# sisl/NeRFSafetyValidation

Measured on AMD Instinct MI355X. Metric: rendered_samples_per_sec, higher is better.
Workload: dtype f16; 1 GPU; Stonehenge 800x800 synthetic, hashgrid L=16 F=2 T=2^19 + ffmlp(64,2)/(64,3), fp16, occupancy-grid ray marching (run_cuda eval path, BASELINE configs[1]); rays_per_frame=640000, bound=2, cascade=2, frames_in_flight=3, fused_reference_rounding=True, parallelism=single GPU, rccl_ranks=1

## Files before the change

nerfsafetyvalidation_amd/csrc/render_fused.hip:

```cpp
#include <hip/hip_fp16.h>
#include <math.h>
#include <string.h>

#include <atomic>
#include <mutex>

#include "ngp_common.hpp"

namespace ngp {

typedef _Float16 half8 __attribute__((ext_vector_type(8)));
typedef _Float16 half2v __attribute__((ext_vector_type(2)));
typedef _Float16 half4 __attribute__((ext_vector_type(4)));
typedef float f32x4 __attribute__((ext_vector_type(4)));

constexpr int kWaves = 8;
constexpr int kThreads = kWaves * 64;
constexpr int kWavesPerSimd = 4;
constexpr int kCh = 2;
constexpr int kSlots = 64 * kCh;
constexpr size_t kLinMaxBytes = 4u << 20;
constexpr size_t kCoarseMaxBytes = 8192;
constexpr int kLookahead = 4;
constexpr int kRing = 8;
// ... 2026 lines not shown
    Pcg32 rng;
    const uint32_t* coarse;
    uint32_t coarse_words;
    const uint32_t* bitfield_lin;
    uint32_t log_grid;
    uint32_t block_jump;
    uint32_t* sample_hash;
    unsigned long long* stamps;
    float2* march_samples;
    uint8_t* march_counts;
    uint32_t wave_slots;
    uint32_t n_rays;
    uint32_t pre_verdict;
    uint32_t wave_march_max;
    uint32_t cell_runs;
};

__host__ __device__ __forceinline__ uint32_t item_width(uint32_t n_alive, uint32_t wave_slots) {
    return n_alive >= 64u * wave_slots ? 64u : (n_alive >= 32u * wave_slots ? 32u : 16u);
}
__device__ __forceinline__ void truncate_launch(Ctl& c, const uint32_t* exhausted, uint32_t N) {
    if (!c.spec) return;
    const uint32_t q = c.spec, K = c.n_step / q;
    uint32_t alive = c.n_alive, ok = K;
    for (uint32_t j = 0; j < K; j++) {
        if (alive == 0) break;
        const uint32_t want_q = N / alive;
        if (j > 0 && (want_q < 1 ? 1u : (want_q > 8 ? 8u : want_q)) != q) { ok = j; break; }
        alive -= exhausted[j] < alive ? exhausted[j] : alive;
    }
// ... 13 lines not shown
    float t[kSlots], dt[kSlots], sig[kSlots];
    uint32_t rg[kSlots], b[kSlots];
    uint16_t list[kSlots];
    float od[64][6];
};

__device__ __forceinline__ void dump_row(const RenderArgs& ra, uint32_t entry, int32_t ray, uint32_t n_step, uint32_t k, float sg, float r,
                                         float g, float b) {
    if (ra.dump_rec) {
        ra.dump_rec[(size_t)ray * 8 + k] = make_float4(sg, r, g, b);
    } else {
        const size_t row = (size_t)entry * n_step + k;
        ra.last_sigmas[row] = sg;
        ra.last_rgbs[row * 3] = r; ra.last_rgbs[row * 3 + 1] = g; ra.last_rgbs[row * 3 + 2] = b;
    }
}

__device__ __forceinline__ void march_ahead_wave(const RenderArgs& ra, float bound, const Ctl& ctl, const uint32_t* coarse) {
    const uint32_t lane = threadIdx.x & 63u;
    const uint32_t entry = blockIdx.x * 4u + (threadIdx.x >> 6);
    if (entry >= ctl.n_alive) return;
    const uint32_t n_step = ctl.n_step, spec = ctl.spec;
    const int32_t ray = ra.alive_in[entry];
    Dda dda;
    dda.init(ra.rays_o + (size_t)ray * 3, ra.rays_d + (size_t)ray * 3, ra.bitfield, bound, 0.0f, ra.max_steps, ra.cascade, ra.grid_size);
    dda.init_lin(ra.bitfield_lin, ra.log_grid, ra.block_jump != 0);
    const float t_c = ra.rays_t[ray], far = ra.fars[ray];
    float t_march = t_c;
    if (ra.perturb) {
        Pcg32 rng = ra.rng;
// ... 162 lines not shown
    if (ctl.spec) {
        uint32_t* exhausted = reinterpret_cast<uint32_t*>(smem);
        if (threadIdx.x < kSpecK) {
            uint32_t d = 0;
            for (int sh = 0; sh < kDeathShards; sh++) d += ra.death_shards[(size_t)kDeathShards * kSpecK + sh * kSpecK + threadIdx.x];
            exhausted[threadIdx.x] = d;
        }
        __syncthreads();
        truncate_launch(ctl, exhausted, ra.n_rays);
        __syncthreads();
    }
    const uint32_t n_alive = ctl.n_alive, n_step = ctl.n_step;
    const uint32_t spec = ctl.spec;
    const uint32_t W = item_width(n_alive, ra.wave_slots);
    const uint32_t n_chunks = (n_alive + W - 1) / W;

    const size_t w_bytes = net_w_bytes_f16(na);
    _Float16* Wlds = reinterpret_cast<_Float16*>(smem);
    LevelTab* lt = reinterpret_cast<LevelTab*>(smem + w_bytes);
    WaveSlab* slabs = reinterpret_cast<WaveSlab*>(smem + w_bytes + sizeof(LevelTab));
    stage_block(na, lv, Wlds, lt, w_bytes);

    const uint32_t lane = threadIdx.x & 63, wid = threadIdx.x >> 6, c = lane & 15;
    WaveSlab& S = slabs[wid];
    unsigned long long ts0 = 0, ts1 = 0;
#define NGP_STAMP(idx)                                                                  \
    if (ra.stamps) {                                                                    \
        ts1 = __builtin_amdgcn_s_memtime();                                             \
        if (lane == 0) atomicAdd(ra.stamps + (idx), ts1 - ts0);                         \
        ts0 = ts1;                                                                      \
// ... 127 lines not shown
                }
                if (lane < 16 && valid) {
                    S.sig[slot] = na.density_scale * sg;
                    S.rg[slot] = (uint32_t)__builtin_bit_cast(uint16_t, (_Float16)r) | ((uint32_t)__builtin_bit_cast(uint16_t, (_Float16)g) << 16);
                    S.b[slot] = (uint32_t)__builtin_bit_cast(uint16_t, (_Float16)b);
                }
            }
            if (ra.stamps && lane == 0) {
                atomicAdd(ra.stamps + 8, sub_a); atomicAdd(ra.stamps + 9, sub_b); atomicAdd(ra.stamps + 10, sub_n); atomicAdd(ra.stamps + 11, sub_f);
            }
            NGP_STAMP(1)
            if (running) {
                uint32_t k = 0;
                for (; k < cnt; k++) {
                    const uint32_t slot = lane * kCh + k;
                    const float dt = S.dt[slot];
                    const float t_after = S.t[slot] + dt;
                    const float delta1 = t_after - last_t;
                    last_t = t_after;
                    const float sg = S.sig[slot];
                    const uint32_t rg = S.rg[slot];
                    const float sr = (float)__builtin_bit_cast(_Float16, (uint16_t)(rg & 0xffffu));
                    const float sgc = (float)__builtin_bit_cast(_Float16, (uint16_t)(rg >> 16));
                    const float sb = (float)__builtin_bit_cast(_Float16, (uint16_t)(S.b[slot] & 0xffffu));
                    const float alpha = 1.0f - expf(-sg * dt);
                    const float T = 1 - ws;
                    const float w = alpha * T;
                    ws += w;
                    t_c += delta1;
                    dep = fmaf(w, t_c, dep);
                    cr = fmaf(w, sr, cr); cg = fmaf(w, sgc, cg); cb = fmaf(w, sb, cb);
                    if (spec && (s0 + k + 1) % spec == 0) last_t = t_c;
                    if ((double)T < 1e-4) break;
                }
                steps_done += k;
                if (k < want) running = false;
            } else if (do_march && cnt) {
                last_t = S.t[lane * kCh + cnt - 1] + S.dt[lane * kCh + cnt - 1];
            }
            if (ra.last_sigmas && active && !spec) {
                for (uint32_t k = 0; k < want; k++) {
                    const uint32_t slot = lane * kCh + k;
                    if (k < cnt)
                        dump_row(ra, entry, ray, n_step, s0 + k, S.sig[slot], (float)__builtin_bit_cast(_Float16, (uint16_t)(S.rg[slot] & 0xffffu)),
                                 (float)__builtin_bit_cast(_Float16, (uint16_t)(S.rg[slot] >> 16)),
                                 (float)__builtin_bit_cast(_Float16, (uint16_t)(S.b[slot] & 0xffffu)));
                    else
                        dump_row(ra, entry, ray, n_step, s0 + k, ra.pad_sigma, ra.pad_r, ra.pad_g, ra.pad_b);
                }
            }
            NGP_STAMP(2)
            if (!ra.last_sigmas && !__any(running)) break;
        }

        const bool survive = active && running && steps_done == n_step;
        if (active) {
            if (survive) ra.rays_t[ray] = t_c;
            if (ra.sample_hash) {
                const uint32_t entered = (spec && !survive) ? (steps_done / spec + 1) * spec : n_step;
                const uint32_t n_hash = emitted < entered ? emitted : entered;
                uint32_t hsh = ra.sample_hash[ray];
                float lm = t_start, gtc = t_c0;
                for (uint32_t i = 0; i < n_hash; i++) {
                    const float2 v = marched[(size_t)i * 64];
                    const float ta = v.x + v.y, d1 = ta - lm;
                    lm = ta;
                    hsh = (hsh ^ __float_as_uint(v.y)) * 16777619u;
                    hsh = (hsh ^ __float_as_uint(d1)) * 16777619u;
                    gtc += d1;
                    if (spec && (i + 1) % spec == 0) lm = gtc;
                }
                ra.sample_hash[ray] = hsh;
            }
            ra.weights_sum[ray] = ws; ra.depth[ray] = dep;
            ra.image[(size_t)ray * 3] = cr; ra.image[(size_t)ray * 3 + 1] = cg; ra.image[(size_t)ray * 3 + 2] = cb;
        }
        const bool slow = ra.sort_slow && survive && slow_next;
        const unsigned long long ball_f = __ballot(survive && !slow), ball_s = __ballot(survive && slow);
        const unsigned long long lt_mask = (1ull << lane) - 1ull;
        if (survive && !slow) ra.staging[(size_t)first_entry + (uint32_t)__popcll(ball_f & lt_mask)] = ray;
        if (survive && slow) ra.staging[(size_t)first_entry + W - 1 - (uint32_t)__popcll(ball_s & lt_mask)] = ray;
        if (lane == 0) ra.chunk_count[chunk] = (uint32_t)__popcll(ball_f) | ((uint32_t)__popcll(ball_s) << 16);
        if (spec) {
            const uint32_t ds = ((blockIdx.x * kWaves + wid) % kDeathShards) * kSpecK;
            for (uint32_t m = 0; m < n_step / spec; m++) {
                const uint32_t cdead = (uint32_t)__popcll(__ballot(active && !survive && steps_done / spec == m));
                if (lane == 0 && cdead) atomicAdd(&ra.death_shards[ds + m], cdead);
            }
        }
        {
            const uint32_t entered = (spec && !survive) ? (steps_done / spec + 1) * spec : n_step;
            uint32_t rm = active ? (emitted < entered ? emitted : entered) : 0u;
#pragma unroll
            for (int off = 32; off > 0; off >>= 1) rm += __shfl_xor(rm, off, 64);
            wave_samples = rm;
        }
        wave_total += wave_samples;
        if (ra.dump_iter && active) ra.dump_iter[ray] = ctl.iters;
        if (ra.last_sigmas && !ra.dump_rec && !spec && chunk == n_chunks - 1) {
            for (uint32_t i = lane; i < 128; i += 64) {
                const size_t row = (size_t)n_alive * n_step + i;
                ra.last_sigmas[row] = ra.pad_sigma;
// ... 10 lines not shown
                                               uint32_t call_tag = 0) {
    if (!host_slot) return;
    if (n.done && fin) {
        const unsigned long long tag = (unsigned long long)(0x8000u | (call_tag & 0x7FFFu)) << 48;
        __hip_atomic_store(fin + 0, tag | (n.samples_marched & 0xFFFFFFFFFFFFull), __ATOMIC_RELAXED, __HIP_MEMORY_SCOPE_SYSTEM);
        __hip_atomic_store(fin + 1, tag | (n.samples_slots & 0xFFFFFFFFFFFFull), __ATOMIC_RELAXED, __HIP_MEMORY_SCOPE_SYSTEM);
        __hip_atomic_store(fin + 2, tag | ((unsigned long long)(n.iters & 0xFFFFFFu) << 24) | (n.rollbacks & 0xFFFFFFu), __ATOMIC_RELAXED,
                           __HIP_MEMORY_SCOPE_SYSTEM);
        __hip_atomic_store(fin + 3, tag | ((unsigned long long)n.last_n_alive << 8) | (n.last_n_step & 0xFFu), __ATOMIC_RELAXED,
                           __HIP_MEMORY_SCOPE_SYSTEM);
    }
    const unsigned long long w = ((unsigned long long)seq << 32) | ((unsigned long long)(n.done ? 1u : 0u) << 31) | (n.n_alive & 0x7FFFFFFFu);
    __hip_atomic_store(host_slot, w, __ATOMIC_RELAXED, __HIP_MEMORY_SCOPE_SYSTEM);
}

__global__ void __launch_bounds__(256) k_render_compact(const Ctl* __restrict__ cur, Ctl* __restrict__ nxt, const int32_t* __restrict__ staging,
                                                         const uint32_t* __restrict__ chunk_count, int32_t* __restrict__ alive_out, uint32_t N,
                                                         uint32_t max_steps, const unsigned long long* __restrict__ stat_shards,
                                                         QueueHeads* __restrict__ nxt_heads, unsigned long long* __restrict__ host_slot, uint32_t seq,
                                                         const uint32_t* __restrict__ death_shards, uint32_t spec_allowed, const int32_t* __restrict__ alive_in,
                                                         const float4* __restrict__ backup, float* __restrict__ rays_t, float* __restrict__ weights_sum,
                                                         float* __restrict__ depth, float* __restrict__ image, uint32_t* __restrict__ sample_hash,
                                                         unsigned long long* stat_shards_rw, uint32_t* __restrict__ death_next, uint32_t wave_slots,
                                                         uint32_t cap_mid_max, uint32_t cap_hi, unsigned long long* __restrict__ fin_host, uint32_t call_tag) {
    __shared__ uint32_t red[3][4];
    __shared__ uint32_t off_f[9], off_s[9];
    Ctl c = *cur;
    if (c.done) {
        if (blockIdx.x == 0 && threadIdx.x == 0) {
            *nxt = c;
            publish_status(host_slot, c, seq, fin_host, call_tag);
        }
        return;
    }
    const uint32_t W = item_width(c.n_alive, wave_slots);
    const uint32_t n_chunks = (c.n_alive + W - 1) / W;
    const uint32_t n_blocks = (n_chunks + 7) / 8;
    const uint32_t g = blockIdx.x;
    if (g >= n_blocks) return;
// ... 18 lines not shown
            const uint32_t q = c.spec, K = c.n_step / q;
            uint32_t alive = c.n_alive;
            keep = K;
            for (uint32_t j = 0; j < K; j++) {
                if (alive == 0) break;
                const uint32_t want_q = N / alive;
                if (j > 0 && (want_q < 1 ? 1u : (want_q > 8 ? 8u : want_q)) != q) { bad = 1; keep = j; break; }
                alive -= deaths[j];
                if ((spec_allowed & 2u) && alive == 0) { bad = 1; keep = j; break; }
            }
        }
        verdict_bad = bad;
        verdict_keep = keep;
    }
    __syncthreads();
    if (verdict_bad) {
        for (uint32_t e = first * W + threadIdx.x; e < (first + 8) * W && e < c.n_alive; e += 256) {
            const int32_t ray = alive_in[e];
            const float4 a = backup[(size_t)ray * 2], b = backup[(size_t)ray * 2 + 1];
            rays_t[ray] = a.x; weights_sum[ray] = a.y; depth[ray] = a.z;
            if (sample_hash) sample_hash[ray] = __float_as_uint(a.w);
            image[(size_t)ray * 3] = b.x; image[(size_t)ray * 3 + 1] = b.y; image[(size_t)ray * 3 + 2] = b.z;
            alive_out[e] = ray;
        }
        if (g == n_blocks - 1 && threadIdx.x == 0) {
            Ctl n = c;
            n.rollbacks = c.rollbacks + 1;
            if (verdict_keep >= 2 && !(spec_allowed & 4u)) {
                n.spec = c.spec;
                n.n_step = verdict_keep * c.spec;
                n.backoff = 0;
                for (uint32_t i = 0; i < kDeathWords; i++) death_next[i] = 0;
            } else {
                n.spec = 0;
                const uint32_t ns = c.n_alive ? N / c.n_alive : 8;
                n.n_step = ns < 1 ? 1 : (ns > 8 ? 8 : ns);
                n.backoff = 2;
            }
            for (int i = 0; i < kStatShards; i++) stat_shards_rw[i] = 0ull;
            *nxt = n;
            for (int i = 0; i < 8; i++) nxt_heads->head[i][0] = 0;
            publish_status(host_slot, n, seq, fin_host, call_tag);
        }
        return;
    }
    uint32_t pf = 0, ps = 0, tf = 0;
    for (uint32_t j = threadIdx.x; j < n_chunks; j += 256) {
        const uint32_t v = chunk_count[j];
        tf += v >> 16;
        if (j < first) { pf += v & 0xffffu; ps += v >> 16; }
    }
#pragma unroll
    for (int off = 32; off > 0; off >>= 1) {
        pf += __shfl_down(pf, off, 64);
// ... 14 lines not shown
    const uint32_t prefix_f = red[0][0] + red[0][1] + red[0][2] + red[0][3];
    const uint32_t prefix_s = red[1][0] + red[1][1] + red[1][2] + red[1][3];
    const uint32_t total_s = red[2][0] + red[2][1] + red[2][2] + red[2][3];
    const uint32_t lane = threadIdx.x & 63, w = threadIdx.x >> 6;
#pragma unroll
    for (uint32_t h = 0; h < 2; h++) {
        const uint32_t ci = w * 2 + h;
        const uint32_t nf = off_f[ci + 1] - off_f[ci], ns = off_s[ci + 1] - off_s[ci];
        if (lane < ns) alive_out[prefix_s + off_s[ci] + lane] = staging[(size_t)(first + ci) * W + W - 1 - lane];
        if (lane < nf) alive_out[total_s + prefix_f + off_f[ci] + lane] = staging[(size_t)(first + ci) * W + lane];
    }
    unsigned long long marched = threadIdx.x < (uint32_t)kStatShards ? stat_shards_rw[threadIdx.x] : 0ull;
#pragma unroll
    for (int off = 32; off > 0; off >>= 1) marched += __shfl_down(marched, off, 64);
    if (g == n_blocks - 1 && threadIdx.x == 0) {
        Ctl n = c;
        n.samples_marched = c.samples_marched + marched;
        for (int i = 0; i < kStatShards; i++) stat_shards_rw[i] = 0ull;
        n.n_alive = total_s + prefix_f + off_f[8];
        uint32_t recent = c.n_alive - n.n_alive;
        if (!c.spec) {
            n.last_n_alive = c.n_alive;
            n.last_n_step = c.n_step;
            n.iters = c.iters + 1;
            n.samples_slots = c.samples_slots + (unsigned long long)c.n_alive * c.n_step;
            n.step = c.step + c.n_step;
        } else {
            const uint32_t q = c.spec, K = c.n_step / q;
            uint32_t alive = c.n_alive, d_last = 0, d_prev = 0;
            unsigned long long slots = c.samples_slots;
            uint32_t it = 0;
            for (uint32_t j = 0; j < K; j++) {
                if (alive == 0) break;
                slots += (unsigned long long)alive * q;
                it++;
                n.last_n_alive = alive;
                n.last_n_step = q;
                alive -= deaths[j];
                d_prev = d_last;
                d_last = deaths[j];
            }
            recent = d_last > d_prev ? d_last : d_prev;
            n.iters = c.iters + it;
            n.samples_slots = slots;
            n.step = c.step + it * q;
        }
        uint32_t ns = n.n_alive ? N / n.n_alive : 8;
        n.n_step = ns < 1 ? 1 : (ns > 8 ? 8 : ns);
        n.done = (n.n_alive == 0 || n.step >= max_steps) ? 1 : 0;
        n.spec = 0;
        if (n.backoff) n.backoff--;
        else if (spec_allowed && !n.done && n.n_step <= kSpecMaxQ && (n.n_step == 8 || n.n_alive > N / (n.n_step + 1))) {
            const uint32_t q = n.n_step;
            const bool own_last = (spec_allowed & 2u) != 0;
            uint32_t room = (max_steps - n.step) / q;
            if (own_last && room) room--;
            const uint32_t headroom = n.n_alive - (q == 8 ? 0u : N / (q + 1)) - 1;
            uint32_t sq = 0;
            while ((unsigned long long)(sq + 1) * (sq + 1) <= recent) sq++;
            const unsigned long long rate = (unsigned long long)recent + 4ull * sq + 16ull;
            const uint32_t safety_x2 = (spec_allowed >> 8) ? (spec_allowed >> 8) : kSpecSafetyX2;
            uint32_t K = (uint32_t)((unsigned long long)headroom * 2u / (safety_x2 * rate));
            const uint32_t cap_mid = 8u * q < cap_mid_max ? 8u * q : cap_mid_max;
            const uint32_t cap_samples = q == 1 ? 8u : (q <= 4 ? cap_mid : cap_hi);
            const uint32_t capK = cap_samples / q < kSpecK ? cap_samples / q : kSpecK;
            K = (q == 8 && !own_last) ? capK : (K < capK ? K : capK);
            K = K < room ? K : room;
            if (K >= 2) { n.spec = q; n.n_step = K * q; }
        }
        if (n.spec)
            for (uint32_t i = 0; i < kDeathWords; i++) death_next[i] = 0;
        *nxt = n;
        for (int i = 0; i < 8; i++) nxt_heads->head[i][0] = 0;
        publish_status(host_slot, n, seq, fin_host, call_tag);
    }
}

__global__ void __launch_bounds__(256) k_render_init(uint32_t N, const float* __restrict__ nears, float* __restrict__ rays_t,
                                                      int32_t* __restrict__ alive, float* __restrict__ weights_sum, float* __restrict__ depth,
                                                      float* __restrict__ image, Ctl* __restrict__ ctl, uint32_t max_steps,
                                                      uint32_t* __restrict__ sample_hash, unsigned long long* __restrict__ stat_shards,
                                                      QueueHeads* __restrict__ heads, uint32_t* __restrict__ death_shards, uint32_t spec_allowed,
                                                      uint32_t tile_w) {
    const uint32_t n = blockIdx.x * 256 + threadIdx.x;
    if (n < (uint32_t)kStatShards) stat_shards[n] = 0ull;
    if (n < 2u * kDeathWords) death_shards[n] = 0;
    if (n < 16) heads[n >> 3].head[n & 7][0] = 0;
    if (n < N) {
        if (sample_hash) sample_hash[n] = 2166136261u;
        uint32_t first = n;
        if (tile_w) {
            const uint32_t t = n >> 4, in = n & 15u, per_row = tile_w >> 2;
            first = ((t / per_row) * 4u + (in >> 2)) * tile_w + (t % per_row) * 4u + (in & 3u);
        }
        alive[n] = (int32_t)first;
        rays_t[n] = nears[n];
        weights_sum[n] = 0; depth[n] = 0;
        image[(size_t)n * 3] = 0; image[(size_t)n * 3 + 1] = 0; image[(size_t)n * 3 + 2] = 0;
    }
    if (n == 0) {
// ... 81 lines not shown
}

using namespace ngp;

struct ngp_render_ctx {
    uint32_t max_rays = 0;
    uint32_t frame_width = 0;
    int32_t* alive[2] = {nullptr, nullptr};
    int32_t* staging = nullptr;
    uint32_t* chunk_count = nullptr;
    float* rays_t = nullptr;
    unsigned long long* coarse = nullptr;
    uint32_t* grid_lin = nullptr;
    uint32_t* death_shards = nullptr;
    float4* backup = nullptr;
    float2* march_samples = nullptr;
    uint8_t* march_counts = nullptr;
    float4* dump_rec = nullptr;
    uint32_t* dump_iter = nullptr;
    Ctl* ctl = nullptr;
    unsigned long long* stat_shards = nullptr;
    QueueHeads* heads = nullptr;
    _Float16* packed = nullptr;
    unsigned long long* status = nullptr;
    unsigned long long* status_dev = nullptr;
    unsigned long long* fin = nullptr;
    unsigned long long* fin_dev = nullptr;
    uint32_t calls = 0;
    uint32_t seq_base = 0;
    hipEvent_t ev[kRing];
// ... 7 lines not shown
struct DebugState {
    int flags = 0;
    unsigned long long* stamps = nullptr;
    uint32_t* sample_hash = nullptr;
    bool coarse_off() const { return (flags & 2) != 0; }
    bool sort_off() const { return (flags & 4) != 0; }
    bool lin_off() const { return (flags & 8) != 0; }
    bool jump_off() const { return (flags & 1) != 0; }
    bool spec_off() const { return (flags & 256) != 0; }
    bool tile_off() const { return (flags & 8192) != 0; }
    bool pre_verdict_off() const { return (flags & 16384) != 0; }
    bool narrow_items_off() const { return (flags & 32768) != 0; }
    bool prefix_replay_off() const { return (flags & 65536) != 0; }
    bool wave_march_off() const { return (flags & 131072) != 0; }
    bool cell_runs_off() const { return (flags & 262144) != 0; }
    uint32_t spec_safety_x2() const { return ((uint32_t)flags >> 9) & 15u; }
    uint32_t shrink() const { return ((uint32_t)flags >> 4) & 15u; }
};
static std::mutex g_debug_mu;
static DebugState g_debug_default;
static float* g_grad_dump = nullptr;
static DebugState debug_snapshot(const ngp_render_ctx* ctx) {
    if (ctx && ctx->has_debug) {
        DebugState d;
        d.flags = ctx->debug_flags; d.stamps = ctx->debug_stamps; d.sample_hash = ctx->debug_sample_hash;
        return d;
    }
    std::lock_guard<std::mutex> lk(g_debug_mu);
    return g_debug_default;
}
// ... 127 lines not shown
    bool ok = true;
    int cus = 256;
    {
        int dev = 0;
        hipDeviceProp_t prop;
        if (hipGetDevice(&dev) == hipSuccess && hipGetDeviceProperties(&prop, dev) == hipSuccess) cus = prop.multiProcessorCount;
    }
    const size_t max_items = items_bound(max_rays, (uint32_t)cus * 16u) + 8;
    ok &= hipMalloc(&c->alive[0], (size_t)max_rays * 4) == hipSuccess;
    ok &= hipMalloc(&c->alive[1], (size_t)max_rays * 4) == hipSuccess;
    ok &= hipMalloc(&c->staging, chunks * 64 * 4) == hipSuccess;
    ok &= hipMalloc(&c->chunk_count, (max_items > (size_t)div_up(max_rays, 256) ? max_items : (size_t)div_up(max_rays, 256)) * 4) == hipSuccess;
    ok &= hipMalloc(&c->rays_t, (size_t)max_rays * 4) == hipSuccess;
    ok &= hipMalloc(&c->coarse, kCoarseMaxBytes) == hipSuccess;
    ok &= hipMalloc(&c->ctl, 2 * sizeof(Ctl)) == hipSuccess;
    ok &= hipMalloc(&c->stat_shards, kStatShards * sizeof(unsigned long long)) == hipSuccess;
    ok &= hipMalloc(&c->death_shards, 2 * (size_t)kDeathWords * sizeof(uint32_t)) == hipSuccess;
    ok &= hipMalloc(&c->backup, (size_t)max_rays * 2 * sizeof(float4)) == hipSuccess;
    ok &= hipMalloc(&c->march_samples, ((size_t)max_rays + 512) * 8 * sizeof(float2)) == hipSuccess;
    ok &= hipMalloc(&c->march_counts, (size_t)max_rays) == hipSuccess;
    ok &= hipMalloc(&c->heads, 2 * sizeof(QueueHeads)) == hipSuccess;
    ok &= hipMalloc(&c->packed, (size_t)(sig_halfs(2) + sig_halfs(3)) * 2) == hipSuccess;
    ok &= hipHostMalloc(&c->status, kRing * sizeof(unsigned long long), hipHostMallocMapped | hipHostMallocCoherent) == hipSuccess;
    if (ok) {
        memset(c->status, 0, kRing * sizeof(unsigned long long));
        ok &= hipHostGetDevicePointer((void**)&c->status_dev, c->status, 0) == hipSuccess;
    }
    ok &= hipHostMalloc(&c->fin, 4 * sizeof(unsigned long long), hipHostMallocMapped | hipHostMallocCoherent) == hipSuccess;
    if (ok) {
        memset(c->fin, 0, 4 * sizeof(unsigned long long));
        ok &= hipHostGetDevicePointer((void**)&c->fin_dev, c->fin, 0) == hipSuccess;
    }
    for (int i = 0; i < kRing; i++) ok &= hipEventCreateWithFlags(&c->ev[i], hipEventDisableTiming) == hipSuccess;
    int dev = 0;
    hipDeviceProp_t prop;
// ... 5 lines not shown
    }
    *out = c;
    return NGP_OK;
}

int ngp_render_ctx_set_frame_width(ngp_render_ctx* ctx, uint32_t width) {
    NGP_REQUIRE(ctx, "render_ctx_set_frame_width: null context");
    ctx->frame_width = width;
    return NGP_OK;
}

int ngp_render_ctx_destroy(ngp_render_ctx* c) {
    if (!c) return NGP_OK;
    (void)hipDeviceSynchronize();
    (void)hipFree(c->alive[0]); (void)hipFree(c->alive[1]); (void)hipFree(c->staging); (void)hipFree(c->chunk_count);
    (void)hipFree(c->rays_t); (void)hipFree(c->coarse); (void)hipFree(c->grid_lin); (void)hipFree(c->death_shards); (void)hipFree(c->backup); (void)hipFree(c->march_samples); (void)hipFree(c->march_counts); (void)hipFree(c->dump_rec); (void)hipFree(c->dump_iter); (void)hipFree(c->ctl); (void)hipFree(c->stat_shards); (void)hipFree(c->heads); (void)hipFree(c->packed);
    if (c->status) (void)hipHostFree(c->status);
    if (c->fin) (void)hipHostFree(c->fin);
    for (int i = 0; i < kRing; i++) (void)hipEventDestroy(c->ev[i]);
    delete c;
    return NGP_OK;
}

static std::atomic<int> g_active_renders{0};
struct ActiveRender {
    ActiveRender() { g_active_renders.fetch_add(1, std::memory_order_relaxed); }
    ~ActiveRender() { g_active_renders.fetch_sub(1, std::memory_order_relaxed); }
};

int ngp_render_rays(ngp_render_ctx* ctx, const ngp_model* model, const float* rays_o, const float* rays_d, const float* nears,
                    const float* fars, uint32_t N, float dt_gamma, uint32_t max_steps, uint32_t perturb, float* weights_sum, float* depth,
// ... 10 lines not shown
    NGP_REQUIRE(model->cascade >= 1 && model->cascade <= 8 && model->grid_size >= 2 && model->grid_size <= 1024,
                "render_rays: unsupported cascade/grid size");
    hipStream_t s = (hipStream_t)stream;
    const DebugState dbg = debug_snapshot(ctx);
    NetArgs na;
    GridLevels lv;
    const _Float16* packed = model && model->packed_weights ? (const _Float16*)model->packed_weights : ctx->packed;
    int rc = fill_net(model, dbg, packed, na, lv);
    if (rc) return rc;
    NGP_REQUIRE(!na.f32(), "render_rays: the occupancy-grid loop is built for the fp16 network (ngp_model::precision == NGP_PREC_F16)");
    if (!model->packed_weights) {
        const uint32_t n_packed = sig_halfs(na.sig_mm) + sig_halfs(na.col_mm);
        k_pack_weights<<<div_up(n_packed, 256), 256, 0, s>>>((const _Float16*)model->sigma_weights, na.sig_mm,
                                                             (const _Float16*)model->color_weights, na.col_mm, ctx->packed);
    }
    const uint32_t spec_allowed = (!dbg.spec_off() && perturb == 0)
                                      ? (1u | (last_sigmas ? 2u : 0u) | (dbg.prefix_replay_off() ? 4u : 0u) | (dbg.spec_safety_x2() << 8)) : 0u;
    const uint32_t fw = ctx->frame_width;
    const uint32_t tile_w = (perturb == 0 && !dbg.tile_off() && fw >= 4 && fw % 4 == 0 && N % (4 * fw) == 0) ? fw : 0u;
    const uint32_t init_threads = N > 2u * kDeathWords ? N : 2u * kDeathWords;
    k_render_init<<<div_up(init_threads, 256), 256, 0, s>>>(N, nears, ctx->rays_t, ctx->alive[0], weights_sum, depth, image, ctx->ctl, max_steps,
                                                 dbg.sample_hash, ctx->stat_shards, ctx->heads, ctx->death_shards, spec_allowed, tile_w);

    RenderArgs ra = {};
    ra.rays_o = rays_o; ra.rays_d = rays_d; ra.fars = fars; ra.rays_t = ctx->rays_t;
    ra.weights_sum = weights_sum; ra.depth = depth; ra.image = image;
    ra.last_sigmas = last_sigmas; ra.last_rgbs = last_rgbs;
    if (pad_value_host) { ra.pad_sigma = pad_value_host[0]; ra.pad_r = pad_value_host[1]; ra.pad_g = pad_value_host[2]; ra.pad_b = pad_value_host[3]; }
    ra.staging = ctx->staging; ra.chunk_count = ctx->chunk_count; ra.stat_shards = ctx->stat_shards;
    {
        static const char* env = getenv("NGP_ITEM_SLOTS");
        ra.wave_slots = dbg.narrow_items_off() ? 0u : (env ? (uint32_t)atoi(env) : (uint32_t)ctx->num_cu * 16u);
        static const bool no_pre = getenv("NGP_NO_PRE_VERDICT") != nullptr;
        ra.pre_verdict = (no_pre || dbg.pre_verdict_off()) ? 0u : 1u;
        static const bool no_runs = getenv("NGP_NO_CELL_RUNS") != nullptr;
        ra.cell_runs = (no_runs || dbg.cell_runs_off()) ? 0u : 1u;
        static const char* wm = getenv("NGP_WAVE_MARCH_MAX");
        ra.wave_march_max = (dbg.wave_march_off() || dt_gamma != 0.0f) ? 0u : (wm ? (uint32_t)atoi(wm) : (uint32_t)ctx->num_cu * 64u);
    }
    ra.backup = ctx->backup;
    ra.march_samples = ctx->march_samples; ra.march_counts = ctx->march_counts;
    ra.bitfield = model->density_bitfield; ra.cascade = model->cascade; ra.grid_size = model->grid_size;
    ra.max_steps = max_steps; ra.perturb = perturb; ra.dt_gamma = dt_gamma;
    ra.n_rays = N;
    ra.rng.seed((uint64_t)perturb);
    ra.stamps = dbg.stamps;
    ra.sort_slow = (perturb == 0 && !dbg.sort_off()) ? 1u : 0u;
    ra.sample_hash = dbg.sample_hash;

    const size_t cells = (size_t)model->cascade * model->grid_size * model->grid_size * model->grid_size;
    const size_t coarse_bytes = cells / 64 / 8;
    const bool use_coarse = !dbg.coarse_off() && cells % 4096 == 0 && coarse_bytes <= kCoarseMaxBytes && ((uintptr_t)model->density_bitfield & 7) == 0;
    const uint32_t Hg = model->grid_size;
    uint32_t logH = 0;
    while ((1u << logH) < Hg) logH++;
// ... 62 lines not shown
        ra.alive_in = ctx->alive[cur];
        ra.ctl = ctx->ctl + cur;
        ra.heads = ctx->heads + cur;
        ra.death_shards = ctx->death_shards + (size_t)cur * kDeathWords;
        {
            ProfScope pm("k_march_ahead", s, 0);
            const uint32_t by_wave = div_up(ub < ra.wave_march_max ? ub : ra.wave_march_max, 4);
            const uint32_t by_lane = div_up(ub ? ub : 1, 256);
            if (lin) k_march_ahead<true><<<by_lane > by_wave ? by_lane : by_wave, 256, 0, s>>>(ra, na.bound);
            else k_march_ahead<false><<<div_up(ub ? ub : 1, 256), 256, 0, s>>>(ra, na.bound);
        }
        {
            ProfScope pk("k_render_iter", s, 0);
            iter_kernel<<<blocks, kThreads, lds, s>>>(na, lv, ra);
        }
        k_render_compact<<<div_up(chunks, 8), 256, 0, s>>>(ctx->ctl + cur, ctx->ctl + (cur ^ 1), ctx->staging, ctx->chunk_count,
                                                           ctx->alive[cur ^ 1], N, max_steps, ctx->stat_shards, ctx->heads + (cur ^ 1),
                                                           ctx->status_dev + launched % kRing, ctx->seq_base + launched + 1,
                                                           ctx->death_shards + (size_t)cur * kDeathWords, spec_allowed, ctx->alive[cur],
                                                           ctx->backup, ctx->rays_t, weights_sum, depth, image, dbg.sample_hash, ctx->stat_shards,
                                                           ctx->death_shards + (size_t)(cur ^ 1) * kDeathWords, ra.wave_slots, cap_mid_max, cap_hi, ctx->fin_dev, call_tag);
        launched++;
        launches += 3;
        while (known < launched) {
            static const uint32_t lookahead = getenv("NGP_LOOKAHEAD") ? (uint32_t)atoi(getenv("NGP_LOOKAHEAD")) : (uint32_t)kLookahead;
            const bool must_wait = launched - known >= lookahead;
            volatile unsigned long long* slot = ctx->status + known % kRing;
            const uint32_t want_seq = ctx->seq_base + known + 1;
            unsigned long long w = *slot;
            if ((uint32_t)(w >> 32) != want_seq) {
                if (!must_wait) break;
                uint32_t spins = 0;
                while ((uint32_t)((w = *slot) >> 32) != want_seq) {
                    if ((++spins & 0xFFFFFu) == 0) {
                        const hipError_t q = hipStreamQuery(s);
                        if (q != hipSuccess && q != hipErrorNotReady) {
// ... 520 lines not shown
```

Before: 7.290 billion samples/s.

## Keep verified speculative prefix on rollback by replaying saved samples

During speculative multi-step iterations, the render kernel now saves each composited sample's sigma and colour plus per-ray step counts and per-chunk survivor counts. When the compact kernel detects a bad speculation verdict, it replays compositing from the backup state over the kept prefix using the saved samples, instead of discarding all speculative work and re-marching. This cuts wasted network evaluations after rollbacks, at the price of extra global writes on every speculative iteration and more buffers. It also adds an env knob for a finer speculation safety factor and factors the state-transition logic into a helper.

New measurement: 7.410 billion samples/s (median of 6 runs). 1.02x the previous value.

```diff
diff --git a/nerfsafetyvalidation_amd/csrc/render_fused.hip b/nerfsafetyvalidation_amd/csrc/render_fused.hip
--- a/nerfsafetyvalidation_amd/csrc/render_fused.hip
+++ b/nerfsafetyvalidation_amd/csrc/render_fused.hip
@@ -2064,6 +2064,10 @@
     uint32_t pre_verdict;
     uint32_t wave_march_max;
     uint32_t cell_runs;
+    uint2* saved_sr;
+    uint16_t* saved_b;
+    uint8_t* steps_done;
+    unsigned long long* item_surv;
 };
 
 __host__ __device__ __forceinline__ uint32_t item_width(uint32_t n_alive, uint32_t wave_slots) {
@@ -2107,6 +2111,37 @@
         ra.last_sigmas[row] = sg;
         ra.last_rgbs[row * 3] = r; ra.last_rgbs[row * 3 + 1] = g; ra.last_rgbs[row * 3 + 2] = b;
     }
+}
+
+__device__ __forceinline__ bool composite_sample(float t, float dt, float sg, uint32_t rg, uint32_t b16, bool boundary, float& last_t, float& t_c,
+                                                 float& ws, float& dep, float& cr, float& cg, float& cb) {
+    const float t_after = t + dt;
+    const float delta1 = t_after - last_t;
+    last_t = t_after;
+    const float sr = (float)__builtin_bit_cast(_Float16, (uint16_t)(rg & 0xffffu));
+    const float sgc = (float)__builtin_bit_cast(_Float16, (uint16_t)(rg >> 16));
+    const float sb = (float)__builtin_bit_cast(_Float16, (uint16_t)(b16 & 0xffffu));
+    const float alpha = 1.0f - expf(-sg * dt);
+    const float T = 1 - ws;
+    const float w = alpha * T;
+    ws += w;
+    t_c += delta1;
+    dep = fmaf(w, t_c, dep);
+    cr = fmaf(w, sr, cr); cg = fmaf(w, sgc, cg); cb = fmaf(w, sb, cb);
+    if (boundary) last_t = t_c;
+    return (double)T < 1e-4;
+}
+__device__ __forceinline__ uint32_t hash_marched(uint32_t hsh, const float2* marched, uint32_t n_hash, uint32_t spec, float lm, float gtc) {
+    for (uint32_t i = 0; i < n_hash; i++) {
+        const float2 v = marched[(size_t)i * 64];
+        const float ta = v.x + v.y, d1 = ta - lm;
+        lm = ta;
+        hsh = (hsh ^ __float_as_uint(v.y)) * 16777619u;
+        hsh = (hsh ^ __float_as_uint(d1)) * 16777619u;
+        gtc += d1;
+        if (spec && (i + 1) % spec == 0) lm = gtc;
+    }
+    return hsh;
 }
 
 __device__ __forceinline__ void march_ahead_wave(const RenderArgs& ra, float bound, const Ctl& ctl, const uint32_t* coarse) {
@@ -2299,6 +2334,7 @@
     const uint32_t spec = ctl.spec;
     const uint32_t W = item_width(n_alive, ra.wave_slots);
     const uint32_t n_chunks = (n_alive + W - 1) / W;
+    const bool save = ra.saved_sr != nullptr && spec != 0 && (spec != 8 || ra.last_sigmas != nullptr);
 
     const size_t w_bytes = net_w_bytes_f16(na);
     _Float16* Wlds = reinterpret_cast<_Float16*>(smem);
@@ -2456,24 +2492,15 @@
                 uint32_t k = 0;
                 for (; k < cnt; k++) {
                     const uint32_t slot = lane * kCh + k;
-                    const float dt = S.dt[slot];
-                    const float t_after = S.t[slot] + dt;
-                    const float delta1 = t_after - last_t;
-                    last_t = t_after;
                     const float sg = S.sig[slot];
-                    const uint32_t rg = S.rg[slot];
-                    const float sr = (float)__builtin_bit_cast(_Float16, (uint16_t)(rg & 0xffffu));
-                    const float sgc = (float)__builtin_bit_cast(_Float16, (uint16_t)(rg >> 16));
-                    const float sb = (float)__builtin_bit_cast(_Float16, (uint16_t)(S.b[slot] & 0xffffu));
-                    const float alpha = 1.0f - expf(-sg * dt);
-                    const float T = 1 - ws;
-                    const float w = alpha * T;
-                    ws += w;
-                    t_c += delta1;
-                    dep = fmaf(w, t_c, dep);
-                    cr = fmaf(w, sr, cr); cg = fmaf(w, sgc, cg); cb = fmaf(w, sb, cb);
-                    if (spec && (s0 + k + 1) % spec == 0) last_t = t_c;
-                    if ((double)T < 1e-4) break;
+                    const uint32_t rg = S.rg[slot], b16 = S.b[slot];
+                    if (save) {
+                        const size_t at = (size_t)(marched - ra.march_samples) + (size_t)(s0 + k) * 64;
+                        ra.saved_sr[at] = make_uint2(__float_as_uint(sg), rg);
+                        ra.saved_b[at] = (uint16_t)b16;
+                    }
+                    if (composite_sample(S.t[slot], S.dt[slot], sg, rg, b16, spec && (s0 + k + 1) % spec == 0, last_t, t_c, ws, dep, cr, cg, cb))
+                        break;
                 }
                 steps_done += k;
                 if (k < want) running = false;
@@ -2501,18 +2528,7 @@
             if (ra.sample_hash) {
                 const uint32_t entered = (spec && !survive) ? (steps_done / spec + 1) * spec : n_step;
                 const uint32_t n_hash = emitted < entered ? emitted : entered;
-                uint32_t hsh = ra.sample_hash[ray];
-                float lm = t_start, gtc = t_c0;
-                for (uint32_t i = 0; i < n_hash; i++) {
-                    const float2 v = marched[(size_t)i * 64];
-                    const float ta = v.x + v.y, d1 = ta - lm;
-                    lm = ta;
-                    hsh = (hsh ^ __float_as_uint(v.y)) * 16777619u;
-                    hsh = (hsh ^ __float_as_uint(d1)) * 16777619u;
-                    gtc += d1;
-                    if (spec && (i + 1) % spec == 0) lm = gtc;
-                }
-                ra.sample_hash[ray] = hsh;
+                ra.sample_hash[ray] = hash_marched(ra.sample_hash[ray], marched, n_hash, spec, t_start, t_c0);
             }
             ra.weights_sum[ray] = ws; ra.depth[ray] = dep;
             ra.image[(size_t)ray * 3] = cr; ra.image[(size_t)ray * 3 + 1] = cg; ra.image[(size_t)ray * 3 + 2] = cb;
@@ -2525,9 +2541,15 @@
         if (lane == 0) ra.chunk_count[chunk] = (uint32_t)__popcll(ball_f) | ((uint32_t)__popcll(ball_s) << 16);
         if (spec) {
             const uint32_t ds = ((blockIdx.x * kWaves + wid) % kDeathShards) * kSpecK;
+            unsigned long long surv = 0ull;
             for (uint32_t m = 0; m < n_step / spec; m++) {
                 const uint32_t cdead = (uint32_t)__popcll(__ballot(active && !survive && steps_done / spec == m));
                 if (lane == 0 && cdead) atomicAdd(&ra.death_shards[ds + m], cdead);
+                if (save) surv |= (unsigned long long)__popcll(__ballot(active && steps_done >= (m + 1) * spec)) << (8 * m);
+            }
+            if (save) {
+                if (active) ra.steps_done[entry] = (uint8_t)steps_done;
+                if (lane == 0) ra.item_surv[chunk] = surv;
             }
         }
         {
@@ -2568,6 +2590,80 @@
     __hip_atomic_store(host_slot, w, __ATOMIC_RELAXED, __HIP_MEMORY_SCOPE_SYSTEM);
 }
 
+struct PrefixKeep {
+    const uint2* saved_sr;
+    const uint16_t* saved_b;
+    const uint8_t* steps_done;
+    const unsigned long long* item_surv;
+    const float2* march_samples;
+    const uint8_t* march_counts;
+    unsigned long long* pend_cur;
+    unsigned long long* pend_next;
+};
+
+__device__ __forceinline__ Ctl next_state(const Ctl& c, uint32_t n_alive_new, unsigned long long marched, const uint32_t* deaths, uint32_t N,
+                                          uint32_t max_steps, uint32_t spec_allowed, uint32_t cap_mid_max, uint32_t cap_hi,
+                                          uint32_t* __restrict__ death_next) {
+    Ctl n = c;
+    n.samples_marched = c.samples_marched + marched;
+    n.n_alive = n_alive_new;
+    uint32_t recent = c.n_alive - n.n_alive;
+    if (!c.spec) {
+        n.last_n_alive = c.n_alive;
+        n.last_n_step = c.n_step;
+        n.iters = c.iters + 1;
+        n.samples_slots = c.samples_slots + (unsigned long long)c.n_alive * c.n_step;
+        n.step = c.step + c.n_step;
+    } else {
+        const uint32_t q = c.spec, K = c.n_step / q;
+        uint32_t alive = c.n_alive, d_last = 0, d_prev = 0;
+        unsigned long long slots = c.samples_slots;
+        uint32_t it = 0;
+        for (uint32_t j = 0; j < K; j++) {
+            if (alive == 0) break;
+            slots += (unsigned long long)alive * q;
+            it++;
+            n.last_n_alive = alive;
+            n.last_n_step = q;
+            alive -= deaths[j];
+            d_prev = d_last;
+            d_last = deaths[j];
+        }
+        recent = d_last > d_prev ? d_last : d_prev;
+        n.iters = c.iters + it;
+        n.samples_slots = slots;
+        n.step = c.step + it * q;
+    }
+    uint32_t ns = n.n_alive ? N / n.n_alive : 8;
+    n.n_step = ns < 1 ? 1 : (ns > 8 ? 8 : ns);
+    n.done = (n.n_alive == 0 || n.step >= max_steps) ? 1 : 0;
+    n.spec = 0;
+    if (n.backoff) n.backoff--;
+    else if (spec_allowed && !n.done && n.n_step <= kSpecMaxQ && (n.n_step == 8 || n.n_alive > N / (n.n_step + 1))) {
+        const uint32_t q = n.n_step;
+        const bool own_last = (spec_allowed & 2u) != 0;
+        uint32_t room = (max_steps - n.step) / q;
+        if (own_last && room) room--;
+        const uint32_t headroom = n.n_alive - (q == 8 ? 0u : N / (q + 1)) - 1;
+        uint32_t sq = 0;
+        while ((unsigned long long)(sq + 1) * (sq + 1) <= recent) sq++;
+        const unsigned long long rate = (unsigned long long)recent + 4ull * sq + 16ull;
+        const uint32_t safety_x2 = ((spec_allowed >> 8) & 15u) ? ((spec_allowed >> 8) & 15u) : kSpecSafetyX2;
+        const uint32_t safety_x8 = (spec_allowed >> 16) & 255u;
+        uint32_t K = safety_x8 ? (uint32_t)((unsigned long long)headroom * 8u / (safety_x8 * rate))
+                               : (uint32_t)((unsigned long long)headroom * 2u / (safety_x2 * rate));
+        const uint32_t cap_mid = 8u * q < cap_mid_max ? 8u * q : cap_mid_max;
+        const uint32_t cap_samples = q == 1 ? 8u : (q <= 4 ? cap_mid : cap_hi);
+        const uint32_t capK = cap_samples / q < kSpecK ? cap_samples / q : kSpecK;
+        K = (q == 8 && !own_last) ? capK : (K < capK ? K : capK);
+        K = K < room ? K : room;
+        if (K >= 2) { n.spec = q; n.n_step = K * q; }
+    }
+    if (n.spec)
+        for (uint32_t i = 0; i < kDeathWords; i++) death_next[i] = 0;
+    return n;
+}
+
 __global__ void __launch_bounds__(256) k_render_compact(const Ctl* __restrict__ cur, Ctl* __restrict__ nxt, const int32_t* __restrict__ staging,
                                                          const uint32_t* __restrict__ chunk_count, int32_t* __restrict__ alive_out, uint32_t N,
                                                          uint32_t max_steps, const unsigned long long* __restrict__ stat_shards,
@@ -2576,7 +2672,8 @@
                                                          const float4* __restrict__ backup, float* __restrict__ rays_t, float* __restrict__ weights_sum,
                                                          float* __restrict__ depth, float* __restrict__ image, uint32_t* __restrict__ sample_hash,
                                                          unsigned long long* stat_shards_rw, uint32_t* __restrict__ death_next, uint32_t wave_slots,
-                                                         uint32_t cap_mid_max, uint32_t cap_hi, unsigned long long* __restrict__ fin_host, uint32_t call_tag) {
+                                                         uint32_t cap_mid_max, uint32_t cap_hi, unsigned long long* __restrict__ fin_host, uint32_t call_tag,
+                                                         PrefixKeep pk) {
     __shared__ uint32_t red[3][4];
     __shared__ uint32_t off_f[9], off_s[9];
     Ctl c = *cur;
@@ -2625,6 +2722,78 @@
         verdict_keep = keep;
     }
     __syncthreads();
+    const uint32_t n_step_marched = cur->n_step;
+    if (verdict_bad && pk.saved_sr && verdict_keep >= 1 && (c.spec != 8 || (spec_allowed & 2u))) {
+        const uint32_t q = c.spec, kq = verdict_keep * q, sh = 8u * (verdict_keep - 1u);
+        uint32_t pf = 0;
+        for (uint32_t j = threadIdx.x; j < first && j < n_chunks; j += 256) pf += (uint32_t)(pk.item_surv[j] >> sh) & 0xffu;
+#pragma unroll
+        for (int off = 32; off > 0; off >>= 1) pf += __shfl_down(pf, off, 64);
+        if ((threadIdx.x & 63) == 0) red[0][threadIdx.x >> 6] = pf;
+        if (threadIdx.x == 0) {
+            uint32_t af = 0;
+            for (uint32_t i = 0; i < 8; i++) {
+                off_f[i] = af;
+                af += (first + i < n_chunks) ? (uint32_t)(pk.item_surv[first + i] >> sh) & 0xffu : 0u;
+            }
+            off_f[8] = af;
+        }
+        __syncthreads();
+        const uint32_t prefix = red[0][0] + red[0][1] + red[0][2] + red[0][3];
+        const uint32_t lane = threadIdx.x & 63, w = threadIdx.x >> 6;
+        uint32_t kept_samples = 0;
+        for (uint32_t h = 0; h < 2; h++) {
+            const uint32_t ci = w * 2 + h, e = (first + ci) * W + lane;
+            const bool valid = lane < W && e < c.n_alive;
+            bool surv = false;
+            int32_t ray = -1;
+            if (valid) {
+                ray = alive_in[e];
+                const uint32_t sd = pk.steps_done[e], em = pk.march_counts[e] & 63u;
+                surv = sd >= kq;
+                const uint32_t entered = surv ? kq : (sd / q + 1) * q;
+                kept_samples += em < entered ? em : entered;
+            }
+            if (surv) {
+                const size_t at = ((size_t)(e >> 6) * n_step_marched) * 64 + (e & 63u);
+                const float2* marched = pk.march_samples + at;
+                const float4 a = backup[(size_t)ray * 2], b = backup[(size_t)ray * 2 + 1];
+                float t_c = a.x, last_t = a.x, ws = a.y, dep = a.z, cr = b.x, cg = b.y, cb = b.z;
+                for (uint32_t i = 0; i < kq; i++) {
+                    const float2 v = marched[(size_t)i * 64];
+                    const uint2 o = pk.saved_sr[at + (size_t)i * 64];
+                    if (composite_sample(v.x, v.y, __uint_as_float(o.x), o.y, pk.saved_b[at + (size_t)i * 64], (i + 1) % q == 0, last_t, t_c, ws, dep,
+                                         cr, cg, cb))
+                        break;
+                }
+                rays_t[ray] = t_c; weights_sum[ray] = ws; depth[ray] = dep;
+                image[(size_t)ray * 3] = cr; image[(size_t)ray * 3 + 1] = cg; image[(size_t)ray * 3 + 2] = cb;
+                if (sample_hash) sample_hash[ray] = hash_marched(__float_as_uint(a.w), marched, kq, q, a.x, a.x);
+            }
+            const unsigned long long ball = __ballot(surv);
+            if (surv) alive_out[prefix + off_f[ci] + (uint32_t)__popcll(ball & ((1ull << lane) - 1ull))] = ray;
+        }
+#pragma unroll
+        for (int off = 32; off > 0; off >>= 1) kept_samples += __shfl_xor(kept_samples, off, 64);
+        if (lane == 0 && kept_samples) atomicAdd(&pk.pend_next[(g * 4u + w) % kStatShards], (unsigned long long)kept_samples);
+        if (g == n_blocks - 1 && threadIdx.x == 0) {
+            Ctl p = c;
+            p.rollbacks = c.rollbacks + 1;
+            if (verdict_keep >= 2) { p.n_step = kq; p.backoff = 0; }
+            else { p.spec = 0; p.n_step = q; p.backoff = 2; }
+            unsigned long long pend = 0ull;
+            for (int i = 0; i < kStatShards; i++) {
+                stat_shards_rw[i] = 0ull;
+                pend += pk.pend_cur[i];
+                pk.pend_cur[i] = 0ull;
+            }
+            const Ctl n = next_state(p, prefix + off_f[8], pend, deaths, N, max_steps, spec_allowed, cap_mid_max, cap_hi, death_next);
+            *nxt = n;
+            for (int i = 0; i < 8; i++) nxt_heads->head[i][0] = 0;
+            publish_status(host_slot, n, seq, fin_host, call_tag);
+        }
+        return;
+    }
     if (verdict_bad) {
         for (uint32_t e = first * W + threadIdx.x; e < (first + 8) * W && e < c.n_alive; e += 256) {
             const int32_t ray = alive_in[e];
@@ -2648,7 +2817,11 @@
                 n.n_step = ns < 1 ? 1 : (ns > 8 ? 8 : ns);
                 n.backoff = 2;
             }
-            for (int i = 0; i < kStatShards; i++) stat_shards_rw[i] = 0ull;
+            for (int i = 0; i < kStatShards; i++) {
+                stat_shards_rw[i] = 0ull;
+                n.samples_marched += pk.pend_cur[i];
+                pk.pend_cur[i] = 0ull;
+            }
             *nxt = n;
             for (int i = 0; i < 8; i++) nxt_heads->head[i][0] = 0;
             publish_status(host_slot, n, seq, fin_host, call_tag);
@@ -2693,62 +2866,8 @@
 #pragma unroll
     for (int off = 32; off > 0; off >>= 1) marched += __shfl_down(marched, off, 64);
     if (g == n_blocks - 1 && threadIdx.x == 0) {
-        Ctl n = c;
-        n.samples_marched = c.samples_marched + marched;
-        for (int i = 0; i < kStatShards; i++) stat_shards_rw[i] = 0ull;
-        n.n_alive = total_s + prefix_f + off_f[8];
-        uint32_t recent = c.n_alive - n.n_alive;
-        if (!c.spec) {
-            n.last_n_alive = c.n_alive;
-            n.last_n_step = c.n_step;
-            n.iters = c.iters + 1;
-            n.samples_slots = c.samples_slots + (unsigned long long)c.n_alive * c.n_step;
-            n.step = c.step + c.n_step;
-        } else {
-            const uint32_t q = c.spec, K = c.n_step / q;
-            uint32_t alive = c.n_alive, d_last = 0, d_prev = 0;
-            unsigned long long slots = c.samples_slots;
-            uint32_t it = 0;
-            for (uint32_t j = 0; j < K; j++) {
-                if (alive == 0) break;
-                slots += (unsigned long long)alive * q;
-                it++;
-                n.last_n_alive = alive;
-                n.last_n_step = q;
-                alive -= deaths[j];
-                d_prev = d_last;
-                d_last = deaths[j];
-            }
-            recent = d_last > d_prev ? d_last : d_prev;
-            n.iters = c.iters + it;
-            n.samples_slots = slots;
-            n.step = c.step + it * q;
-        }
-        uint32_t ns = n.n_alive ? N / n.n_alive : 8;
-        n.n_step = ns < 1 ? 1 : (ns > 8 ? 8 : ns);
-        n.done = (n.n_alive == 0 || n.step >= max_steps) ? 1 : 0;
-        n.spec = 0;
-        if (n.backoff) n.backoff--;
-        else if (spec_allowed && !n.done && n.n_step <= kSpecMaxQ && (n.n_step == 8 || n.n_alive > N / (n.n_step + 1))) {
-            const uint32_t q = n.n_step;
-            const bool own_last = (spec_allowed & 2u) != 0;
-            uint32_t room = (max_steps - n.step) / q;
-            if (own_last && room) room--;
-            const uint32_t headroom = n.n_alive - (q == 8 ? 0u : N / (q + 1)) - 1;
-            uint32_t sq = 0;
-            while ((unsigned long long)(sq + 1) * (sq + 1) <= recent) sq++;
-            const unsigned long long rate = (unsigned long long)recent + 4ull * sq + 16ull;
-            const uint32_t safety_x2 = (spec_allowed >> 8) ? (spec_allowed >> 8) : kSpecSafetyX2;
-            uint32_t K = (uint32_t)((unsigned long long)headroom * 2u / (safety_x2 * rate));
-            const uint32_t cap_mid = 8u * q < cap_mid_max ? 8u * q : cap_mid_max;
-            const uint32_t cap_samples = q == 1 ? 8u : (q <= 4 ? cap_mid : cap_hi);
-            const uint32_t capK = cap_samples / q < kSpecK ? cap_samples / q : kSpecK;
-            K = (q == 8 && !own_last) ? capK : (K < capK ? K : capK);
-            K = K < room ? K : room;
-            if (K >= 2) { n.spec = q; n.n_step = K * q; }
-        }
-        if (n.spec)
-            for (uint32_t i = 0; i < kDeathWords; i++) death_next[i] = 0;
+        for (int i = 0; i < kStatShards; i++) { stat_shards_rw[i] = 0ull; marched += pk.pend_cur[i]; pk.pend_cur[i] = 0ull; }
+        const Ctl n = next_state(c, total_s + prefix_f + off_f[8], marched, deaths, N, max_steps, spec_allowed, cap_mid_max, cap_hi, death_next);
         *nxt = n;
         for (int i = 0; i < 8; i++) nxt_heads->head[i][0] = 0;
         publish_status(host_slot, n, seq, fin_host, call_tag);
@@ -2762,7 +2881,7 @@
                                                       QueueHeads* __restrict__ heads, uint32_t* __restrict__ death_shards, uint32_t spec_allowed,
                                                       uint32_t tile_w) {
     const uint32_t n = blockIdx.x * 256 + threadIdx.x;
-    if (n < (uint32_t)kStatShards) stat_shards[n] = 0ull;
+    if (n < 3u * kStatShards) stat_shards[n] = 0ull;
     if (n < 2u * kDeathWords) death_shards[n] = 0;
     if (n < 16) heads[n >> 3].head[n & 7][0] = 0;
     if (n < N) {
@@ -2874,6 +2993,10 @@
     uint32_t* grid_lin = nullptr;
     uint32_t* death_shards = nullptr;
     float4* backup = nullptr;
+    uint2* saved_sr = nullptr;
+    uint16_t* saved_b = nullptr;
+    uint8_t* steps_done = nullptr;
+    unsigned long long* item_surv = nullptr;
     float2* march_samples = nullptr;
     uint8_t* march_counts = nullptr;
     float4* dump_rec = nullptr;
@@ -2911,6 +3034,7 @@
     bool prefix_replay_off() const { return (flags & 65536) != 0; }
     bool wave_march_off() const { return (flags & 131072) != 0; }
     bool cell_runs_off() const { return (flags & 262144) != 0; }
+    bool prefix_keep_off() const { return (flags & 524288) != 0; }
     uint32_t spec_safety_x2() const { return ((uint32_t)flags >> 9) & 15u; }
     uint32_t shrink() const { return ((uint32_t)flags >> 4) & 15u; }
 };
@@ -3068,11 +3192,15 @@
     ok &= hipMalloc(&c->rays_t, (size_t)max_rays * 4) == hipSuccess;
     ok &= hipMalloc(&c->coarse, kCoarseMaxBytes) == hipSuccess;
     ok &= hipMalloc(&c->ctl, 2 * sizeof(Ctl)) == hipSuccess;
-    ok &= hipMalloc(&c->stat_shards, kStatShards * sizeof(unsigned long long)) == hipSuccess;
+    ok &= hipMalloc(&c->stat_shards, 3 * kStatShards * sizeof(unsigned long long)) == hipSuccess;
     ok &= hipMalloc(&c->death_shards, 2 * (size_t)kDeathWords * sizeof(uint32_t)) == hipSuccess;
     ok &= hipMalloc(&c->backup, (size_t)max_rays * 2 * sizeof(float4)) == hipSuccess;
     ok &= hipMalloc(&c->march_samples, ((size_t)max_rays + 512) * 8 * sizeof(float2)) == hipSuccess;
     ok &= hipMalloc(&c->march_counts, (size_t)max_rays) == hipSuccess;
+    ok &= hipMalloc(&c->saved_sr, ((size_t)max_rays + 512) * 8 * sizeof(uint2)) == hipSuccess;
+    ok &= hipMalloc(&c->saved_b, ((size_t)max_rays + 512) * 8 * sizeof(uint16_t)) == hipSuccess;
+    ok &= hipMalloc(&c->steps_done, (size_t)max_rays) == hipSuccess;
+    ok &= hipMalloc(&c->item_surv, max_items * sizeof(unsigned long long)) == hipSuccess;
     ok &= hipMalloc(&c->heads, 2 * sizeof(QueueHeads)) == hipSuccess;
     ok &= hipMalloc(&c->packed, (size_t)(sig_halfs(2) + sig_halfs(3)) * 2) == hipSuccess;
     ok &= hipHostMalloc(&c->status, kRing * sizeof(unsigned long long), hipHostMallocMapped | hipHostMallocCoherent) == hipSuccess;
@@ -3108,7 +3236,7 @@
     if (!c) return NGP_OK;
     (void)hipDeviceSynchronize();
     (void)hipFree(c->alive[0]); (void)hipFree(c->alive[1]); (void)hipFree(c->staging); (void)hipFree(c->chunk_count);
-    (void)hipFree(c->rays_t); (void)hipFree(c->coarse); (void)hipFree(c->grid_lin); (void)hipFree(c->death_shards); (void)hipFree(c->backup); (void)hipFree(c->march_samples); (void)hipFree(c->march_counts); (void)hipFree(c->dump_rec); (void)hipFree(c->dump_iter); (void)hipFree(c->ctl); (void)hipFree(c->stat_shards); (void)hipFree(c->heads); (void)hipFree(c->packed);
+    (void)hipFree(c->rays_t); (void)hipFree(c->coarse); (void)hipFree(c->grid_lin); (void)hipFree(c->death_shards); (void)hipFree(c->backup); (void)hipFree(c->march_samples); (void)hipFree(c->march_counts); (void)hipFree(c->saved_sr); (void)hipFree(c->saved_b); (void)hipFree(c->steps_done); (void)hipFree(c->item_surv); (void)hipFree(c->dump_rec); (void)hipFree(c->dump_iter); (void)hipFree(c->ctl); (void)hipFree(c->stat_shards); (void)hipFree(c->heads); (void)hipFree(c->packed);
     if (c->status) (void)hipHostFree(c->status);
     if (c->fin) (void)hipHostFree(c->fin);
     for (int i = 0; i < kRing; i++) (void)hipEventDestroy(c->ev[i]);
@@ -3149,8 +3277,10 @@
         k_pack_weights<<<div_up(n_packed, 256), 256, 0, s>>>((const _Float16*)model->sigma_weights, na.sig_mm,
                                                              (const _Float16*)model->color_weights, na.col_mm, ctx->packed);
     }
+    static const uint32_t safety_x8_env = getenv("NGP_SPEC_SAFETY_X8") ? ((uint32_t)atoi(getenv("NGP_SPEC_SAFETY_X8")) & 255u) : 0u;
     const uint32_t spec_allowed = (!dbg.spec_off() && perturb == 0)
-                                      ? (1u | (last_sigmas ? 2u : 0u) | (dbg.prefix_replay_off() ? 4u : 0u) | (dbg.spec_safety_x2() << 8)) : 0u;
+                                      ? (1u | (last_sigmas ? 2u : 0u) | (dbg.prefix_replay_off() ? 4u : 0u) | (dbg.spec_safety_x2() << 8) |
+                                         (safety_x8_env << 16)) : 0u;
     const uint32_t fw = ctx->frame_width;
     const uint32_t tile_w = (perturb == 0 && !dbg.tile_off() && fw >= 4 && fw % 4 == 0 && N % (4 * fw) == 0) ? fw : 0u;
     const uint32_t init_threads = N > 2u * kDeathWords ? N : 2u * kDeathWords;
@@ -3174,6 +3304,9 @@
         ra.wave_march_max = (dbg.wave_march_off() || dt_gamma != 0.0f) ? 0u : (wm ? (uint32_t)atoi(wm) : (uint32_t)ctx->num_cu * 64u);
     }
     ra.backup = ctx->backup;
+    if (!dbg.prefix_keep_off() && !dbg.prefix_replay_off()) {
+        ra.saved_sr = ctx->saved_sr; ra.saved_b = ctx->saved_b; ra.steps_done = ctx->steps_done; ra.item_surv = ctx->item_surv;
+    }
     ra.march_samples = ctx->march_samples; ra.march_counts = ctx->march_counts;
     ra.bitfield = model->density_bitfield; ra.cascade = model->cascade; ra.grid_size = model->grid_size;
     ra.max_steps = max_steps; ra.perturb = perturb; ra.dt_gamma = dt_gamma;
@@ -3266,12 +3399,14 @@
             ProfScope pk("k_render_iter", s, 0);
             iter_kernel<<<blocks, kThreads, lds, s>>>(na, lv, ra);
         }
+        const PrefixKeep pk = {ra.saved_sr, ra.saved_b, ra.steps_done, ra.item_surv, ra.march_samples, ra.march_counts,
+                               ctx->stat_shards + (size_t)(1 + cur) * kStatShards, ctx->stat_shards + (size_t)(2 - cur) * kStatShards};
         k_render_compact<<<div_up(chunks, 8), 256, 0, s>>>(ctx->ctl + cur, ctx->ctl + (cur ^ 1), ctx->staging, ctx->chunk_count,
                                                            ctx->alive[cur ^ 1], N, max_steps, ctx->stat_shards, ctx->heads + (cur ^ 1),
                                                            ctx->status_dev + launched % kRing, ctx->seq_base + launched + 1,
                                                            ctx->death_shards + (size_t)cur * kDeathWords, spec_allowed, ctx->alive[cur],
                                                            ctx->backup, ctx->rays_t, weights_sum, depth, image, dbg.sample_hash, ctx->stat_shards,
-                                                           ctx->death_shards + (size_t)(cur ^ 1) * kDeathWords, ra.wave_slots, cap_mid_max, cap_hi, ctx->fin_dev, call_tag);
+                                                           ctx->death_shards + (size_t)(cur ^ 1) * kDeathWords, ra.wave_slots, cap_mid_max, cap_hi, ctx->fin_dev, call_tag, pk);
         launched++;
         launches += 3;
         while (known < launched) {
```
